# magnate3/dpdk_dc_sand

Hardware: AMD Instinct MI355X
Metric: int8 voltage Gsamples/s ingested + beams/s, 64-ant 4096-ch; % HBM roofline (higher is better)
Workload: dtype int8

## Files before the change

### dpdk_dc_sand_amd/csrc/bf_wide_i8.hip

```cpp
#include <algorithm>
#include <cstdlib>
#include <type_traits>

#include "bf_fused.hpp"

namespace bf {

namespace {

constexpr int kW8Threads = 256;

__device__ __forceinline__ int w8_step_base(int s, int A) { return min(32 * s, A - 32); }
__host__ __device__ inline int w8_padded_steps(int A) { return 2 * ((((A + 31) >> 5) + 1) / 2); }


__host__ __device__ inline int w32_steps(int A) { return w32_table_steps(A); }

typedef uint16_t u16x2_t __attribute__((ext_vector_type(2)));

__device__ __forceinline__ void w32_expand_unit(int8_t* lb, int ml, int g, const u32x4_t& q0, const u32x4_t& q1) {
  const uint32_t d[8] = {q0[0], q0[1], q0[2], q0[3], q1[0], q1[1], q1[2], q1[3]};
  uint32_t n[8], np[8], pp[8];
#pragma unroll
  for (int i = 0; i < 8; ++i) {
    const u16x2_t v = __builtin_bit_cast(u16x2_t, d[i]);
    const u16x2_t neg = v * u16x2_t{1, 0xffff};
    n[i] = __builtin_bit_cast(uint32_t, neg);
    np[i] = __builtin_bit_cast(uint32_t, neg + u16x2_t{128, 128});
    pp[i] = __builtin_bit_cast(uint32_t, v + u16x2_t{128, 128});
  }
  u32x4_t e_hi0, e_lo0, e_hi1, e_lo1;
#pragma unroll
  for (int q = 0; q < 4; ++q) {
    e_lo0[q] = __builtin_amdgcn_perm(n[2 * q + 1], n[2 * q], 0x06040200u);
    e_hi0[q] = __builtin_amdgcn_perm(np[2 * q + 1], np[2 * q], 0x07050301u);
    e_lo1[q] = __builtin_amdgcn_perm(d[2 * q + 1], d[2 * q], 0x04060002u);
    e_hi1[q] = __builtin_amdgcn_perm(pp[2 * q + 1], pp[2 * q], 0x05070103u);
  }
  const int st = g >> 2, h = g & 3, tau = ml >> 3, row = (2 * ml) & 15;
  int8_t* o = lb + ((((st * 4 + tau) * 2) * 64) + row + 16 * h) * 16;
  *reinterpret_cast<u32x4_t*>(o) = e_hi0;
  *reinterpret_cast<u32x4_t*>(o + 64 * 16) = e_lo0;
  *reinterpret_cast<u32x4_t*>(o + 16) = e_hi1;
  *reinterpret_cast<u32x4_t*>(o + 16 + 64 * 16) = e_lo1;
}

__device__ __forceinline__ void w32_load(const uint8_t* __restrict__ base, size_t ant_stride, uint32_t loff, int s,
                                         int A, u32x2_t (&d)[8]) {
  const int a0 = w8_step_base(s, A);
#pragma unroll
  for (int q = 0; q < 8; ++q)
    d[q] = *reinterpret_cast<const u32x2_t*>(base + static_cast<size_t>(a0 + q) * ant_stride + loff);
}

__device__ __forceinline__ void w32_load_buf(__amdgpu_buffer_rsrc_t rs, uint32_t voff, uint32_t sbase, uint32_t stride,
                                             u32x2_t (&d)[8]) {
#pragma unroll
  for (int q = 0; q < 8; ++q)
    d[q] = __builtin_bit_cast(u32x2_t, __builtin_amdgcn_raw_buffer_load_b64(rs, voff, sbase + q * stride, 0));
}

template <bool Signed>
__device__ __forceinline__ void w32_frags(const u32x2_t (&d)[8], i32x4_t (&f)[2][2]) {
#pragma unroll
  for (int p = 0; p < 2; ++p)
#pragma unroll
    for (int i = 0; i < 2; ++i) {
      uint32_t w[4];
#pragma unroll
      for (int m2 = 0; m2 < 4; ++m2) {
        const u32x2_t da = d[2 * m2], db = d[2 * m2 + 1];
        uint32_t a = i ? da.y : da.x, b = i ? db.y : db.x;
        if constexpr (!Signed) {
          a ^= 0x80808080u;
          b ^= 0x80808080u;
        }
        w[m2] = __builtin_amdgcn_perm(b, a, p ? kSelP1 : kSelP0);
      }
      f[p][i] = i32x4_t{static_cast<int>(w[0]), static_cast<int>(w[1]), static_cast<int>(w[2]), static_cast<int>(w[3])};
    }
}

__device__ __forceinline__ void w32_mfma(const int4* __restrict__ fr, int s, int lane, const i32x4_t (&f)[2][2],
                                         i32x4_t (&hi)[2][2][4], i32x4_t (&lo)[2][2][4]) {
#pragma unroll
  for (int t = 0; t < 4; ++t) {
    const int4 x0 = fr[(((s * 4 + t) * 2 + 0) * 64) + lane];
    const int4 x1 = fr[(((s * 4 + t) * 2 + 1) * 64) + lane];
    const i32x4_t chi = i32x4_t{x0.x, x0.y, x0.z, x0.w}, clo = i32x4_t{x1.x, x1.y, x1.z, x1.w};
#pragma unroll
    for (int p = 0; p < 2; ++p)
#pragma unroll
      for (int i = 0; i < 2; ++i) {
        hi[p][i][t] = mfma_i8(chi, f[p][i], hi[p][i][t]);
        lo[p][i][t] = mfma_i8(clo, f[p][i], lo[p][i][t]);
      }
  }
}

template <bool Signed, bool Gain = false>
__global__ __launch_bounds__(kW8Threads, 2) void beamform_fused_i8_w32_kernel(FusedArgs P) {
  extern __shared__ __attribute__((aligned(16))) int4 lds4[];
  const int tid = threadIdx.x, lane = tid & 63, wave = tid >> 6;
  const int h = lane >> 4, tl = lane & 15;
  int slab, bc;
  if (P.xcd_order) {
    const int x = blockIdx.x & 7, local = blockIdx.x >> 3;
    slab = local % P.nslabs;
    bc = (local / P.nslabs) * 8 + x;
    if (bc >= P.B * P.C) return;
  } else {
    slab = blockIdx.x % P.nslabs;
    bc = blockIdx.x / P.nslabs;
  }
  const int b = bc / P.C, c = bc % P.C;
  const int m0 = slab * kW32Beams;
  const int Sp = w32_steps(P.A);
  const int T2 = P.T >> 1;
  const int nchunks = (T2 + 15) >> 4;
  const int npasses = (nchunks + 3) >> 2;
  const size_t ant_stride = static_cast<size_t>(P.C) * P.T * 4;
  const uint32_t hoff = static_cast<uint32_t>(8 * h) * static_cast<uint32_t>(ant_stride);
  const uint8_t* base = P.raw + (static_cast<size_t>(b) * P.A * P.C + c) * static_cast<size_t>(P.T) * 4;
  int8_t* lb = reinterpret_cast<int8_t*>(lds4);
  int* partial = reinterpret_cast<int*>(lb + static_cast<size_t>(Sp) * 4 * 2 * 64 * 16);

  __builtin_assume(Sp >= 4 && (Sp & 3) == 0 && npasses >= 1);
  const int total = npasses * Sp;
  int issued = 0, ls = 0, lchunk = wave;
  auto issue = [&](u32x2_t (&d)[8]) {
    const uint32_t loff = hoff + static_cast<uint32_t>(min(lchunk * 16 + tl, T2 - 1)) * 8u;
    w32_load(base, ant_stride, loff, ls, P.A, d);
    ++issued;
    const bool adv = issued < total;
    const bool wrap = ls + 1 == Sp;
    ls = adv ? (wrap ? 0 : ls + 1) : ls;
    lchunk = (adv && wrap) ? lchunk + 4 : lchunk;
  };
  const int ml = (tid >> 2) & (kW32Beams - 1);
  const int sa0 = 4 * (tid >> 7) + (tid & 3);
  const bool m_ok = m0 + ml < P.M;
  const float4* dv_row =
      P.dv + (static_cast<size_t>(P.delay_channels == 1 ? 0 : c) * P.M + min(m0 + ml, P.M - 1)) * P.A;
  const float* g_row = Gain ? P.gain + static_cast<size_t>(min(m0 + ml, P.M - 1)) * P.A : nullptr;
  constexpr int kBatch = 8;
  auto batch_model = [&](int j0, float4 (&dv)[kBatch], float (&gv)[kBatch]) {
#pragma unroll
    for (int j = 0; j < kBatch; ++j) {
      const int sa = sa0 + 8 * (j0 + j), st = sa >> 5;
      const int a = min(w8_step_base(st, P.A) + (sa & 31), P.A - 1);
      dv[j] = dv_row[a];
      if constexpr (Gain)
        gv[j] = g_row[a];
      else
        gv[j] = 1.0f;
    }
  };
  float4 dv_first[kBatch];
  float gv_first[kBatch];
  batch_model(0, dv_first, gv_first);
  __builtin_amdgcn_sched_barrier(0);

  u32x2_t d0[8], d1[8], d2[8], d3[8];
  issue(d0);
  issue(d1);
  issue(d2);
  issue(d3);
  __builtin_amdgcn_sched_barrier(0);

  {
    const double dt = P.t0 + static_cast<double>(b) * P.batch_dt;
    const double ch = static_cast<double>(P.base_ch + c);
    const int nj = 4 * Sp;
    int cs0 = 0, cs1 = 0;
    const int off0 = coef8_byte(2 * sa0, 2 * ml, 4, 0);
    float4 dv[kBatch];
    float gv[kBatch];
#pragma unroll
    for (int j = 0; j < kBatch; ++j) {
      dv[j] = dv_first[j];
      gv[j] = gv_first[j];
    }
    for (int j0 = 0; j0 < nj; j0 += kBatch) {
      float4 dvn[kBatch];
      float gvn[kBatch];
      batch_model(j0 + kBatch, dvn, gvn);
      bool valid[kBatch];
      int wc[kBatch], ws[kBatch];
#pragma unroll
      for (int j = 0; j < kBatch; ++j) {
        const int sa = sa0 + 8 * (j0 + j), st = sa >> 5;
        const int a = w8_step_base(st, P.A) + (sa & 31);
        valid[j] = j0 + j < nj && m_ok && a >= 32 * st;
      }
      q14_coeffs<kBatch, true>(dv, gv, valid, ch, P.ctot, P.ts, P.k, dt, P.gain, wc, ws);
#pragma unroll
      for (int j = 0; j < kBatch; ++j) {
        if (j0 + j >= nj) break;
        const int J = j0 + j;
        const int Wc = wc[j], Ws = ws[j], nWs = -Ws;
        int8_t* o = lb + off0 + 8192 * (J >> 2) + 256 * (J & 3);
        *reinterpret_cast<uint16_t*>(o) = static_cast<uint16_t>(__builtin_amdgcn_perm(nWs + 128, Wc + 128, 0x0c0c0501u));
        *reinterpret_cast<uint16_t*>(o + 64 * 16) = static_cast<uint16_t>(__builtin_amdgcn_perm(nWs, Wc, 0x0c0c0400u));
        *reinterpret_cast<uint16_t*>(o + 16) = static_cast<uint16_t>(__builtin_amdgcn_perm(Wc + 128, Ws + 128, 0x0c0c0501u));
        *reinterpret_cast<uint16_t*>(o + 16 + 64 * 16) = static_cast<uint16_t>(__builtin_amdgcn_perm(Wc, Ws, 0x0c0c0400u));
        cs0 += Wc - Ws;
        cs1 += Ws + Wc;
      }
#pragma unroll
      for (int j = 0; j < kBatch; ++j) {
        dv[j] = dvn[j];
        gv[j] = gvn[j];
      }
    }
    if constexpr (!Signed) {
      cs0 += __shfl_xor(cs0, 1);
      cs1 += __shfl_xor(cs1, 1);
      cs0 += __shfl_xor(cs0, 2);
      cs1 += __shfl_xor(cs1, 2);
      if ((lane & 3) == 0) {
        partial[wave * 32 + 2 * (lane >> 2)] = cs0;
        partial[wave * 32 + 2 * (lane >> 2) + 1] = cs1;
      }
    }
  }
  lds_barrier();

  const float s32 = P.out_scale * 0x1p-14f;
  const int M2 = 2 * P.M;
  const bool full = m0 + kW32Beams <= P.M && (M2 & 15) == 0;
  int chunk = wave;
  for (int pass = 0; pass < npasses; ++pass) {
    const int tq = chunk * 16 + tl;
    i32x4_t hi[2][2][4], lo[2][2][4];
#pragma unroll
    for (int p = 0; p < 2; ++p)
#pragma unroll
      for (int i = 0; i < 2; ++i)
#pragma unroll
        for (int t = 0; t < 4; ++t) hi[p][i][t] = lo[p][i][t] = i32x4_t{0, 0, 0, 0};
    for (int s = 0; s < Sp; s += 4) {
      i32x4_t f[2][2];
      w32_frags<Signed>(d0, f);
      issue(d0);
      w32_mfma(lds4, s, lane, f, hi, lo);
      w32_frags<Signed>(d1, f);
      issue(d1);
      w32_mfma(lds4, s + 1, lane, f, hi, lo);
      w32_frags<Signed>(d2, f);
      issue(d2);
      w32_mfma(lds4, s + 2, lane, f, hi, lo);
      w32_frags<Signed>(d3, f);
      issue(d3);
      w32_mfma(lds4, s + 3, lane, f, hi, lo);
    }
#pragma unroll
    for (int p = 0; p < 2; ++p) {
      uint32_t pk[2][4];
#pragma unroll
      for (int i = 0; i < 2; ++i)
#pragma unroll
        for (int t = 0; t < 4; ++t) {
          uint32_t qb[4];
#pragma unroll
          for (int r = 0; r < 4; ++r) {
            int y = (hi[p][i][t][r] << 8) + lo[p][i][t][r];
            if constexpr (!Signed) {
              const int cl = 16 * t + 4 * h + r;
              y += 128 * (partial[(cl >> 5) * 32 + (cl & 31)] + partial[((cl >> 5) + 2) * 32 + (cl & 31)]);
            }
            qb[r] = requant_bits(y, s32);
          }
          pk[i][t] = pack_low_bytes(qb[0], qb[1], qb[2], qb[3]);
        }
      const size_t prow = ((static_cast<size_t>(b) * 2 + p) * P.C + c) * static_cast<size_t>(P.T);
      if (full) {
#pragma unroll
        for (int i = 0; i < 2; ++i) transpose_rows4(pk[i]);
        if (tq < T2) {
#pragma unroll
          for (int i = 0; i < 2; ++i) {
            int8_t* o = reinterpret_cast<int8_t*>(P.y) + (prow + 2 * tq + i) * M2 + 2 * m0 + 16 * h;
            *reinterpret_cast<u32x4_t*>(o) = u32x4_t{pk[i][0], pk[i][1], pk[i][2], pk[i][3]};
          }
        }
      } else if (tq < T2) {
#pragma unroll
        for (int i = 0; i < 2; ++i) {
          int8_t* o = reinterpret_cast<int8_t*>(P.y) + (prow + 2 * tq + i) * M2 + 2 * m0;
#pragma unroll
          for (int t = 0; t < 4; ++t)
#pragma unroll
            for (int r = 0; r < 4; ++r) {
              const int col = 16 * t + 4 * h + r;
              if (2 * m0 + col < M2) o[col] = static_cast<int8_t>((pk[i][t] >> (8 * r)) & 255);
            }
        }
      }
    }
    chunk += 4;
  }
}



template <bool Signed, bool Early = true, int kSp = 0, int kNP = 0, int kNB = 4, int kCh = kW32TChannels,
          bool BufLd = false, bool Pow2 = false>
__global__ __launch_bounds__(kW8Threads, 2) void beamform_fused_i8_w32t_kernel(FusedArgs P) {
  extern __shared__ __attribute__((aligned(16))) int4 lds4[];
  const int tid = threadIdx.x, lane = tid & 63, wave = tid >> 6;
  const int h = lane >> 4, tl = lane & 15;
  const int Cn = P.c_count ? P.c_count : P.C;
  const int gpb = (Cn + kCh - 1) / kCh;
  int slab, grp;
  if (P.xcd_order) {
    const int x = blockIdx.x & 7, local = blockIdx.x >> 3;
    slab = local % P.nslabs;
    grp = (local / P.nslabs) * 8 + x;
    if (grp >= P.B * gpb) return;
  } else {
    slab = blockIdx.x % P.nslabs;
    grp = blockIdx.x / P.nslabs;
  }
  const int b = grp / gpb, c0 = (grp - b * gpb) * kCh;
  const int nk = min(kCh, Cn - c0);
  const int m0 = slab * kW32Beams;
  const int Sp = kSp ? kSp : w32_steps(P.A);
  const int T2 = P.T >> 1;
  const int nchunks = (T2 + 15) >> 4;
  const int npasses = kNP ? kNP : (nchunks + 3) >> 2;
  const size_t ant_stride = static_cast<size_t>(P.C) * P.T * 4;
  const uint32_t hoff = static_cast<uint32_t>(8 * h) * static_cast<uint32_t>(ant_stride);
  const uint32_t ch_bytes = static_cast<uint32_t>(P.T) * 4;
  const uint8_t* base = P.raw + (static_cast<size_t>(b) * P.A * P.C + c0) * static_cast<size_t>(P.T) * 4;
  int8_t* lb = reinterpret_cast<int8_t*>(lds4);
  int* partial = reinterpret_cast<int*>(lb + static_cast<size_t>(Sp) * 4 * 2 * 64 * 16);
  const u32x4_t* tbase = reinterpret_cast<const u32x4_t*>(P.table) +
                         ((static_cast<size_t>(b) * P.C + c0) * P.nslabs + slab) * 256 * Sp;
  const size_t tstride = static_cast<size_t>(P.nslabs) * 256 * Sp;

  __builtin_assume(Sp >= 4 && (Sp & 3) == 0 && npasses >= 1 && nk >= 1);
  const int total = nk * npasses * Sp;
  int issued = 0, ls = 0, lp = 0, lk = 0;
  const __amdgpu_buffer_rsrc_t vrs = __builtin_amdgcn_make_buffer_rsrc(const_cast<uint8_t*>(base), 0, 0x7fffffff,
                                                                        0x00020000);
  auto issue = [&](u32x2_t (&d)[8]) {
    if constexpr (BufLd) {
      const uint32_t voff = hoff + static_cast<uint32_t>(min((wave + 4 * lp) * 16 + tl, T2 - 1)) * 8u;
      const uint32_t sbase = static_cast<uint32_t>(w8_step_base(ls, P.A)) * static_cast<uint32_t>(ant_stride) +
                             static_cast<uint32_t>(lk) * ch_bytes;
      w32_load_buf(vrs, voff, sbase, static_cast<uint32_t>(ant_stride), d);
    } else {
      const uint32_t loff = hoff + static_cast<uint32_t>(lk) * ch_bytes +
                            static_cast<uint32_t>(min((wave + 4 * lp) * 16 + tl, T2 - 1)) * 8u;
      w32_load(base, ant_stride, loff, ls, P.A, d);
    }
    ++issued;
    const bool adv = issued < total;
    const bool wrap = ls + 1 == Sp, pwrap = lp + 1 == npasses;
    ls = adv ? (wrap ? 0 : ls + 1) : ls;
    lp = (adv && wrap) ? (pwrap ? 0 : lp + 1) : lp;
    lk = (adv && wrap && pwrap) ? lk + 1 : lk;
  };
  u32x4_t tq[4][2];
  auto load_table = [&](int kc) {
    const __amdgpu_buffer_rsrc_t rs = __builtin_amdgcn_make_buffer_rsrc(
        const_cast<u32x4_t*>(tbase + static_cast<size_t>(kc) * tstride), 0, 0x7fffffff, 0x00020000);
#pragma unroll
    for (int j = 0; j < 4; ++j)
#pragma unroll
      for (int hf = 0; hf < 2; ++hf)
        tq[j][hf] = __builtin_bit_cast(u32x4_t, __builtin_amdgcn_raw_buffer_load_b128(
                                                    rs, static_cast<uint32_t>(((min(j, Sp / 2 - 1) * 2 + hf) * 256 + tid) * 16), 0, 0));
  };
  load_table(0);
  __builtin_amdgcn_sched_barrier(0);
  constexpr int NB = kSp ? kNB : 2;
  u32x2_t db[NB][8];
#pragma unroll
  for (int j = 0; j < NB; ++j) issue(db[j]);
  __builtin_amdgcn_sched_barrier(0);

  const float s32 = P.out_scale * 0x1p-14f;
  const int M2 = 2 * P.M;
  const bool full = m0 + kW32Beams <= P.M && (M2 & 15) == 0;
  for (int kc = 0; kc < nk; ++kc) {
    const int c = c0 + kc;
    {
      const int ml = tid & 31;
      int cs0 = 0, cs1 = 0;
#pragma unroll
      for (int j = 0; j < 4; ++j) {
        if (2 * j >= Sp) break;
        w32_expand_unit(lb, ml, (tid >> 5) + 8 * j, tq[j][0], tq[j][1]);
        if constexpr (!Signed) {
#pragma unroll
          for (int hf = 0; hf < 2; ++hf)
#pragma unroll
            for (int q = 0; q < 4; ++q) {
              const int wc = static_cast<int16_t>(tq[j][hf][q] & 0xffffu), ws = static_cast<int>(tq[j][hf][q]) >> 16;
              cs0 += wc - ws;
              cs1 += ws + wc;
            }
        }
      }
      if constexpr (!Signed) {
        cs0 += __shfl_xor(cs0, 32);
        cs1 += __shfl_xor(cs1, 32);
        if (lane < 32) {
          partial[wave * 64 + 2 * ml] = cs0;
          partial[wave * 64 + 2 * ml + 1] = cs1;
        }
      }
    }
    lds_barrier();
    if constexpr (!Signed) {
      if (tid < 64) partial[tid] += partial[64 + tid] + partial[128 + tid] + partial[192 + tid];
      lds_barrier();
    }
    auto run_pass = [&](int pass, auto last) {
      constexpr bool kLast = decltype(last)::value;
      const int tq2 = (wave + 4 * pass) * 16 + tl;
      i32x4_t hi[2][2][4], lo[2][2][4];
#pragma unroll
      for (int p = 0; p < 2; ++p)
#pragma unroll
        for (int i = 0; i < 2; ++i)
#pragma unroll
          for (int t = 0; t < 4; ++t) hi[p][i][t] = lo[p][i][t] = i32x4_t{0, 0, 0, 0};
      if constexpr (kSp != 0) {
#pragma unroll
        for (int s = 0; s < kSp; ++s) {
          i32x4_t f[2][2];
          const int j = (pass * kSp + s) % NB;
          w32_frags<Signed>(db[j], f);
          __builtin_amdgcn_sched_barrier(0);
          issue(db[j]);
          w32_mfma(lds4, s, lane, f, hi, lo);
          __builtin_amdgcn_sched_barrier(0);
        }
      } else {
        for (int s = 0; s < Sp; s += 2) {
          i32x4_t f[2][2];
#pragma unroll
          for (int j = 0; j < 2; ++j) {
            w32_frags<Signed>(db[j], f);
            issue(db[j]);
            w32_mfma(lds4, s + j, lane, f, hi, lo);
          }
        }
      }
      constexpr bool next_table = kLast && Early;
#pragma unroll
      for (int p = 0; p < 2; ++p) {
        if constexpr (next_table)
          if (p == 1) {
            __builtin_amdgcn_sched_barrier(0);
            load_table(min(kc + 1, nk - 1));
            __builtin_amdgcn_sched_barrier(0);
          }
        uint32_t pk[2][4];
#pragma unroll
        for (int i = 0; i < 2; ++i)
#pragma unroll
          for (int t = 0; t < 4; ++t) {
            uint32_t qb[4];
            int4 cs = int4{0, 0, 0, 0};
            if constexpr (!Signed) cs = reinterpret_cast<const int4*>(partial)[4 * t + h];
            const int csr[4] = {cs.x, cs.y, cs.z, cs.w};
#pragma unroll
            for (int r = 0; r < 4; ++r) {
              int y = (hi[p][i][t][r] << 8) + lo[p][i][t][r];
              if constexpr (!Signed) y += 128 * csr[r];
              qb[r] = requant_bits<Pow2>(y, s32);
            }
            pk[i][t] = pack_low_bytes(qb[0], qb[1], qb[2], qb[3]);
          }
        const size_t prow = ((static_cast<size_t>(b) * 2 + p) * P.C + c) * static_cast<size_t>(P.T);
        if (full) {
#pragma unroll
          for (int i = 0; i < 2; ++i) transpose_rows4(pk[i]);
          if (tq2 < T2) {
#pragma unroll
            for (int i = 0; i < 2; ++i) {
              int8_t* o = reinterpret_cast<int8_t*>(P.y) + (prow + 2 * tq2 + i) * M2 + 2 * m0 + 16 * h;
              *reinterpret_cast<u32x4_t*>(o) = u32x4_t{pk[i][0], pk[i][1], pk[i][2], pk[i][3]};
            }
          }
        } else if (tq2 < T2) {
#pragma unroll
          for (int i = 0; i < 2; ++i) {
            int8_t* o = reinterpret_cast<int8_t*>(P.y) + (prow + 2 * tq2 + i) * M2 + 2 * m0;
#pragma unroll
            for (int t = 0; t < 4; ++t)
#pragma unroll
              for (int r = 0; r < 4; ++r) {
                const int col = 16 * t + 4 * h + r;
                if (2 * m0 + col < M2) o[col] = static_cast<int8_t>((pk[i][t] >> (8 * r)) & 255);
              }
          }
        }
      }
    };
    if constexpr (Early) {
      if constexpr (kNP != 0) {
#pragma unroll
        for (int pass = 0; pass + 1 < kNP; ++pass) run_pass(pass, std::false_type{});
      } else {
        for (int pass = 0; pass + 1 < npasses; ++pass) run_pass(pass, std::false_type{});
      }
      run_pass(npasses - 1, std::true_type{});
    } else {
      if constexpr (kNP != 0) {
#pragma unroll
        for (int pass = 0; pass < kNP; ++pass) run_pass(pass, std::false_type{});
      } else {
        for (int pass = 0; pass < npasses; ++pass) run_pass(pass, std::false_type{});
      }
      load_table(min(kc + 1, nk - 1));
    }
    if constexpr (kSp != 0 && (kSp * kNP) % NB != 0) {
      constexpr int r = (kSp * kNP) % NB;
      u32x2_t tmp[NB][8];
#pragma unroll
      for (int j = 0; j < NB; ++j)
#pragma unroll
        for (int q = 0; q < 8; ++q) tmp[j][q] = db[(j + r) % NB][q];
#pragma unroll
      for (int j = 0; j < NB; ++j)
#pragma unroll
        for (int q = 0; q < 8; ++q) db[j][q] = tmp[j][q];
    }
    if (kc + 1 < nk) lds_barrier();
  }
}

__shared__ __attribute__((aligned(16))) int4 w32r_img[8 * 2 * 2 * 64];
__shared__ __attribute__((aligned(16))) int4 w32r_slot0[4 * 256];
__shared__ __attribute__((aligned(16))) int4 w32r_slot1[4 * 256];
__shared__ __attribute__((aligned(16))) int w32r_ws[4 * 32];

typedef __attribute__((address_space(3))) void* lds_void_ptr;

__device__ __forceinline__ void w32r_expand_unit(int4* img, int ml, int g, const u32x4_t& q0, const u32x4_t& q1) {
  const uint32_t d[8] = {q0[0], q0[1], q0[2], q0[3], q1[0], q1[1], q1[2], q1[3]};
  uint32_t n[8], np[8];
#pragma unroll
  for (int i = 0; i < 8; ++i) {
    const u16x2_t neg = __builtin_bit_cast(u16x2_t, d[i]) * u16x2_t{1, 0xffff};
    n[i] = __builtin_bit_cast(uint32_t, neg);
    np[i] = __builtin_bit_cast(uint32_t, neg + u16x2_t{128, 128});
  }
  u32x4_t ehi, elo;
#pragma unroll
  for (int q = 0; q < 4; ++q) {
    elo[q] = __builtin_amdgcn_perm(n[2 * q + 1], n[2 * q], 0x06040200u);
    ehi[q] = __builtin_amdgcn_perm(np[2 * q + 1], np[2 * q], 0x07050301u);
  }
  int4* o = img + ((g >> 2) * 2 + (ml >> 4)) * 2 * 64 + (ml & 15) + 16 * (g & 3);
  o[0] = __builtin_bit_cast(int4, ehi);
  o[64] = __builtin_bit_cast(int4, elo);
}

__device__ __forceinline__ i32x4_t w32r_frag_im(const i32x4_t& f) {
  i32x4_t r;
#pragma unroll
  for (int q = 0; q < 4; ++q) {
    const uint32_t n = static_cast<uint32_t>(f[q]) ^ 0x00ff00ffu;
    r[q] = static_cast<int>(__builtin_amdgcn_perm(n, n, 0x02030001u));
  }
  return r;
}

template <bool Pow2>
__global__ __launch_bounds__(kW8Threads, 2) void beamform_fused_i8_w32r_kernel(FusedArgs P) {
  constexpr int Sp = 8, NP = 2, kCh = kW32RChannels;
  const int tid = threadIdx.x, lane = tid & 63;
  const int wave = __builtin_amdgcn_readfirstlane(tid >> 6);
  const int h = lane >> 4, tl = lane & 15;
  const int C = P.C;
  const int gpb = (C + kCh - 1) / kCh;
  int slab, grp;
  if (P.xcd_order) {
    const int x = blockIdx.x & 7, local = blockIdx.x >> 3;
    slab = local % P.nslabs;
    grp = (local / P.nslabs) * 8 + x;
    if (grp >= P.B * gpb) return;
  } else {
    slab = blockIdx.x % P.nslabs;
    grp = blockIdx.x / P.nslabs;
  }
  const int b = grp / gpb, c0 = (grp - b * gpb) * kCh;
  const int nk = min(kCh, C - c0);
  const int m0 = slab * kW32Beams;
  const uint32_t ant_stride = static_cast<uint32_t>(C) * static_cast<uint32_t>(P.T) * 4u;
  const uint32_t ch_bytes = static_cast<uint32_t>(P.T) * 4u;
  const uint8_t* base = P.raw + (static_cast<size_t>(b) * P.A * C + c0) * static_cast<size_t>(P.T) * 4;
  const __amdgpu_buffer_rsrc_t vrs = __builtin_amdgcn_make_buffer_rsrc(const_cast<uint8_t*>(base), 0, 0x7fffffff,
                                                                        0x00020000);
  const uint32_t dma_voff = static_cast<uint32_t>(8 * ((lane >> 3) & 3) + (lane >> 5)) * ant_stride +
                            16u * static_cast<uint32_t>(lane & 7);
  int4* const slot0 = w32r_slot0 + 256 * wave;
  int4* const slot1 = w32r_slot1 + 256 * wave;

  const int total = nk * NP * Sp;
  int issued = 0, ls = 0, lp = 0, lk = 0;
  auto dma_sb = [&]() {
    return __builtin_amdgcn_readfirstlane(static_cast<uint32_t>(w8_step_base(ls, P.A)) * ant_stride +
                                          static_cast<uint32_t>(lk) * ch_bytes +
                                          static_cast<uint32_t>(wave + 4 * lp) * 128u);
  };
  auto dma_piece = [&](int4* slot, int k, uint32_t sb) {
    __builtin_amdgcn_raw_ptr_buffer_load_lds(vrs, (lds_void_ptr)(slot + 64 * k), 16, dma_voff,
                                             sb + 2u * static_cast<uint32_t>(k) * ant_stride, 0, 0);
  };
  auto advance = [&]() {
    ++issued;
    const bool adv = issued < total;
    const bool wrap = ls + 1 == Sp, pwrap = lp + 1 == NP;
    ls = adv ? (wrap ? 0 : ls + 1) : ls;
    lp = (adv && wrap) ? (pwrap ? 0 : lp + 1) : lp;
    lk = (adv && wrap && pwrap) ? lk + 1 : lk;
  };
  auto dma = [&](int4* slot) {
    const uint32_t sb = dma_sb();
#pragma unroll
    for (int k = 0; k < 4; ++k) dma_piece(slot, k, sb);
    advance();
  };
  auto read_slot = [&](const int4* slot, u32x2_t (&d)[8]) {
    const u32x2_t* s2 = reinterpret_cast<const u32x2_t*>(slot);
#pragma unroll
    for (int q = 0; q < 8; ++q) d[q] = s2[(4 * q + h) * 16 + tl];
  };

  const u32x4_t* tbase = reinterpret_cast<const u32x4_t*>(P.table) +
                         ((static_cast<size_t>(b) * C + c0) * P.nslabs + slab) * 256 * Sp;
  const size_t tstride = static_cast<size_t>(P.nslabs) * 256 * Sp;
  u32x4_t tq[4][2];
  auto load_table = [&](int kc) {
    const __amdgpu_buffer_rsrc_t rs = __builtin_amdgcn_make_buffer_rsrc(
        const_cast<u32x4_t*>(tbase + static_cast<size_t>(kc) * tstride), 0, 0x7fffffff, 0x00020000);
#pragma unroll
    for (int j = 0; j < 4; ++j)
#pragma unroll
      for (int hf = 0; hf < 2; ++hf)
        tq[j][hf] = __builtin_bit_cast(
            u32x4_t, __builtin_amdgcn_raw_buffer_load_b128(rs, static_cast<uint32_t>(((j * 2 + hf) * 256 + tid) * 16), 0, 0));
  };
  auto expand = [&]() {
    const int ml = tid & 31;
    int ws = 0;
#pragma unroll
    for (int j = 0; j < 4; ++j) {
      w32r_expand_unit(w32r_img, ml, (tid >> 5) + 8 * j, tq[j][0], tq[j][1]);
#pragma unroll
      for (int hf = 0; hf < 2; ++hf)
#pragma unroll
        for (int q = 0; q < 4; ++q) ws += static_cast<int>(tq[j][hf][q]) >> 16;
    }
    ws += __shfl_xor(ws, 32);
    if (lane < 32) w32r_ws[32 * wave + ml] = ws;
  };

  load_table(0);
  __builtin_amdgcn_sched_barrier(0);
  dma(slot0);
  dma(slot1);
  __builtin_amdgcn_sched_barrier(0);
  expand();
  lds_barrier();

  const float s32 = P.out_scale * 0x1p-14f;
  const int M2 = 2 * P.M;
  const __amdgpu_buffer_rsrc_t yrs = __builtin_amdgcn_make_buffer_rsrc(P.y, 0, 0x7fffffff, 0x00020000);
  const uint32_t so_lane = static_cast<uint32_t>(2 * tl * M2 + 16 * (h >> 1) + 32 * (h & 1));
  for (int kc = 0; kc < nk; ++kc) {
    const int c = c0 + kc;
#pragma unroll
    for (int pass = 0; pass < NP; ++pass) {
      i32x4_t rh[2][2][2], rl[2][2][2], ih[2][2][2], il[2][2][2];
#pragma unroll
      for (int p = 0; p < 2; ++p)
#pragma unroll
        for (int i = 0; i < 2; ++i)
#pragma unroll
          for (int t = 0; t < 2; ++t) rh[p][i][t] = rl[p][i][t] = ih[p][i][t] = il[p][i][t] = i32x4_t{0, 0, 0, 0};
#pragma unroll
      for (int s = 0; s < Sp; ++s) {
        int4* const slot = (s & 1) ? slot1 : slot0;
        u32x2_t d[8];
        read_slot(slot, d);
        i32x4_t f[2][2], fi[2][2];
        w32_frags<true>(d, f);
#pragma unroll
        for (int p = 0; p < 2; ++p)
#pragma unroll
          for (int i = 0; i < 2; ++i) fi[p][i] = w32r_frag_im(f[p][i]);
        asm volatile("" ::"v"(f[0][0]), "v"(f[0][1]), "v"(f[1][0]), "v"(f[1][1]) : "memory");
        __builtin_amdgcn_sched_barrier(0);
        const uint32_t sb = dma_sb();
#pragma unroll
        for (int t = 0; t < 2; ++t) {
          const int4 x0 = w32r_img[((s * 2 + t) * 2 + 0) * 64 + lane];
          const int4 x1 = w32r_img[((s * 2 + t) * 2 + 1) * 64 + lane];
          const i32x4_t ahi = i32x4_t{x0.x, x0.y, x0.z, x0.w}, alo = i32x4_t{x1.x, x1.y, x1.z, x1.w};
#pragma unroll
          for (int p = 0; p < 2; ++p) {
            __builtin_amdgcn_sched_barrier(0);
            dma_piece(slot, 2 * t + p, sb);
            __builtin_amdgcn_sched_barrier(0);
#pragma unroll
            for (int i = 0; i < 2; ++i) {
              rh[p][i][t] = mfma_i8(ahi, f[p][i], rh[p][i][t]);
              rl[p][i][t] = mfma_i8(alo, f[p][i], rl[p][i][t]);
              ih[p][i][t] = mfma_i8(ahi, fi[p][i], ih[p][i][t]);
              il[p][i][t] = mfma_i8(alo, fi[p][i], il[p][i][t]);
            }
          }
        }
        advance();
        __builtin_amdgcn_sched_barrier(0);
      }
      if (pass == NP - 1) {
        __builtin_amdgcn_sched_barrier(0);
        load_table(min(kc + 1, nk - 1));
        __builtin_amdgcn_sched_barrier(0);
      }
      int bias[2][4];
#pragma unroll
      for (int t = 0; t < 2; ++t) {
        int4 acc = int4{0, 0, 0, 0};
#pragma unroll
        for (int w = 0; w < 4; ++w) {
          const int4 v = *reinterpret_cast<const int4*>(w32r_ws + 32 * w + 16 * t + 4 * h);
          acc.x += v.x;
          acc.y += v.y;
          acc.z += v.z;
          acc.w += v.w;
        }
        bias[t][0] = -acc.x;
        bias[t][1] = -acc.y;
        bias[t][2] = -acc.z;
        bias[t][3] = -acc.w;
      }
#pragma unroll
      for (int p = 0; p < 2; ++p) {
        const uint32_t prow = static_cast<uint32_t>(((b * 2 + p) * C + c) * P.T);
#pragma unroll
        for (int i = 0; i < 2; ++i) {
          uint32_t pk[2][2];
#pragma unroll
          for (int t = 0; t < 2; ++t) {
            uint32_t qr[4], qi[4];
#pragma unroll
            for (int r = 0; r < 4; ++r) {
              qr[r] = requant_bits<Pow2>((rh[p][i][t][r] << 8) + rl[p][i][t][r], s32);
              qi[r] = requant_bits<Pow2>((ih[p][i][t][r] << 8) + il[p][i][t][r] + bias[t][r], s32);
            }
            pk[t][0] = pack_low_bytes(qr[0], qi[0], qr[1], qi[1]);
            pk[t][1] = pack_low_bytes(qr[2], qi[2], qr[3], qi[3]);
          }
          const auto sw0 = __builtin_amdgcn_permlane16_swap(pk[0][0], pk[1][0], false, false);
          const auto sw1 = __builtin_amdgcn_permlane16_swap(pk[0][1], pk[1][1], false, false);
          const u32x4_t sd = u32x4_t{sw0[0], sw1[0], sw0[1], sw1[1]};
          const uint32_t soff = (prow + static_cast<uint32_t>(2 * (wave + 4 * pass) * 16 + i)) * static_cast<uint32_t>(M2) +
                                static_cast<uint32_t>(2 * m0);
          __builtin_amdgcn_raw_buffer_store_b128(sd, yrs, so_lane, soff, 0);
          __builtin_amdgcn_sched_barrier(0);
          asm volatile("s_nop 1");
          __builtin_amdgcn_sched_barrier(0);
        }
      }
    }
    if (kc + 1 < nk) {
      lds_barrier();
      expand();
      lds_barrier();
    }
  }
  asm volatile("s_waitcnt vmcnt(0)" ::: "memory");
}

template <bool Signed>
FusedKernel w32_kernel(const FusedPlan& p) {
  if constexpr (Signed)
    if (p.family == FusedFamily::W32R)
      return with_bools([](auto pow2) -> FusedKernel { return beamform_fused_i8_w32r_kernel<pow2.value>; }, p.pow2);
  if (p.family == FusedFamily::W32T) {
    if (p.straight)
      return with_bools([](auto pow2) -> FusedKernel {
        return beamform_fused_i8_w32t_kernel<Signed, false, 8, 2, 2, 8, true, pow2.value>;
      }, p.pow2);
    return with_bools([](auto buf) -> FusedKernel {
      return beamform_fused_i8_w32t_kernel<Signed, false, 0, 0, 4, kW32TChannels, buf.value, false>;
    }, p.buf);
  }
  return with_bools([](auto gain) -> FusedKernel { return beamform_fused_i8_w32_kernel<Signed, gain.value>; }, p.gain);
}

}

int launch_w32(const FusedPlan& p, FusedArgs P, hipStream_t st) {
  if (p.table) {
    const int e = launch_q14_table(P, const_cast<uint32_t*>(P.table), kLayoutW32, st);
    if (e != BF_OK) return e;
  }
  return launch_planned(!p.sgn ? w32_kernel<false>(p) : w32_kernel<true>(p), p, P, st);
}

}
```

Measured before the change: 2473.

## Derive DMA indices from counter, fold table offsets into immediates, defer table prefetch

Replaces the incremental ls/lp/lk DMA counters with values decoded from a single issued counter using masks and shifts. Moves the table load's per-slice offset into the instruction's immediate offset, and hides tid behind an opaque asm so the compiler cannot materialise many address registers. Swaps the shuffle for permlane32_swap and moves the next-table prefetch into the epilogue after the first p iteration. The aim is lower register pressure and fewer address calculations, which should help occupancy and scheduling. The decode hardcodes Sp=8 and NP=2 through the shifts and masks, so it is only correct for those values.

After: 2475, median of 6. No clear change (+0.1%).

```diff
diff --git a/dpdk_dc_sand_amd/csrc/bf_wide_i8.hip b/dpdk_dc_sand_amd/csrc/bf_wide_i8.hip
--- a/dpdk_dc_sand_amd/csrc/bf_wide_i8.hip
+++ b/dpdk_dc_sand_amd/csrc/bf_wide_i8.hip
@@ -604,8 +604,9 @@
   int4* const slot1 = w32r_slot1 + 256 * wave;
 
   const int total = nk * NP * Sp;
-  int issued = 0, ls = 0, lp = 0, lk = 0;
+  int issued = 0;
   auto dma_sb = [&]() {
+    const int n = min(issued, total - 1), ls = n & (Sp - 1), lp = (n >> 3) & (NP - 1), lk = n >> 4;
     return __builtin_amdgcn_readfirstlane(static_cast<uint32_t>(w8_step_base(ls, P.A)) * ant_stride +
                                           static_cast<uint32_t>(lk) * ch_bytes +
                                           static_cast<uint32_t>(wave + 4 * lp) * 128u);
@@ -614,14 +615,7 @@
     __builtin_amdgcn_raw_ptr_buffer_load_lds(vrs, (lds_void_ptr)(slot + 64 * k), 16, dma_voff,
                                              sb + 2u * static_cast<uint32_t>(k) * ant_stride, 0, 0);
   };
-  auto advance = [&]() {
-    ++issued;
-    const bool adv = issued < total;
-    const bool wrap = ls + 1 == Sp, pwrap = lp + 1 == NP;
-    ls = adv ? (wrap ? 0 : ls + 1) : ls;
-    lp = (adv && wrap) ? (pwrap ? 0 : lp + 1) : lp;
-    lk = (adv && wrap && pwrap) ? lk + 1 : lk;
-  };
+  auto advance = [&]() { ++issued; };
   auto dma = [&](int4* slot) {
     const uint32_t sb = dma_sb();
 #pragma unroll
@@ -638,7 +632,13 @@
                          ((static_cast<size_t>(b) * C + c0) * P.nslabs + slab) * 256 * Sp;
   const size_t tstride = static_cast<size_t>(P.nslabs) * 256 * Sp;
   u32x4_t tq[4][2];
+  auto opaque_tid = [&]() {
+    int t = tid;
+    asm volatile("" : "+v"(t));
+    return t;
+  };
   auto load_table = [&](int kc) {
+    const int t = opaque_tid();
     const __amdgpu_buffer_rsrc_t rs = __builtin_amdgcn_make_buffer_rsrc(
         const_cast<u32x4_t*>(tbase + static_cast<size_t>(kc) * tstride), 0, 0x7fffffff, 0x00020000);
 #pragma unroll
@@ -646,21 +646,22 @@
 #pragma unroll
       for (int hf = 0; hf < 2; ++hf)
         tq[j][hf] = __builtin_bit_cast(
-            u32x4_t, __builtin_amdgcn_raw_buffer_load_b128(rs, static_cast<uint32_t>(((j * 2 + hf) * 256 + tid) * 16), 0, 0));
+            u32x4_t, __builtin_amdgcn_raw_buffer_load_b128(rs, static_cast<uint32_t>(t * 16), (j * 2 + hf) * 4096, 0));
   };
   auto expand = [&]() {
-    const int ml = tid & 31;
+    const int t = opaque_tid();
+    const int ml = t & 31;
     int ws = 0;
 #pragma unroll
     for (int j = 0; j < 4; ++j) {
-      w32r_expand_unit(w32r_img, ml, (tid >> 5) + 8 * j, tq[j][0], tq[j][1]);
+      w32r_expand_unit(w32r_img + 512 * j, ml, t >> 5, tq[j][0], tq[j][1]);
 #pragma unroll
       for (int hf = 0; hf < 2; ++hf)
 #pragma unroll
         for (int q = 0; q < 4; ++q) ws += static_cast<int>(tq[j][hf][q]) >> 16;
     }
-    ws += __shfl_xor(ws, 32);
-    if (lane < 32) w32r_ws[32 * wave + ml] = ws;
+    ws += static_cast<int>(__builtin_amdgcn_permlane32_swap(ws, ws, false, false)[1]);
+    if ((t & 63) < 32) w32r_ws[32 * wave + ml] = ws;
   };
 
   load_table(0);
@@ -722,18 +723,14 @@
         advance();
         __builtin_amdgcn_sched_barrier(0);
       }
-      if (pass == NP - 1) {
-        __builtin_amdgcn_sched_barrier(0);
-        load_table(min(kc + 1, nk - 1));
-        __builtin_amdgcn_sched_barrier(0);
-      }
       int bias[2][4];
+      const int* const ws_h = w32r_ws + 4 * ((opaque_tid() >> 4) & 3);
 #pragma unroll
       for (int t = 0; t < 2; ++t) {
         int4 acc = int4{0, 0, 0, 0};
 #pragma unroll
         for (int w = 0; w < 4; ++w) {
-          const int4 v = *reinterpret_cast<const int4*>(w32r_ws + 32 * w + 16 * t + 4 * h);
+          const int4 v = *reinterpret_cast<const int4*>(ws_h + 32 * w + 16 * t);
           acc.x += v.x;
           acc.y += v.y;
           acc.z += v.z;
@@ -746,6 +743,11 @@
       }
 #pragma unroll
       for (int p = 0; p < 2; ++p) {
+        if (pass == NP - 1 && p == 1) {
+          __builtin_amdgcn_sched_barrier(0);
+          load_table(min(kc + 1, nk - 1));
+          __builtin_amdgcn_sched_barrier(0);
+        }
         const uint32_t prow = static_cast<uint32_t>(((b * 2 + p) * C + c) * P.T);
 #pragma unroll
         for (int i = 0; i < 2; ++i) {
```
